# arkworks-rs/gemini

Hardware: AMD Instinct MI355X
Metric: BLS12-381 G1 MSM throughput (higher is better)
Workload: dtype u32x12 Montgomery Fq (381-bit integer), u32x8 Fr; 1 GPU; 2^20 G1 MSM per GPU (BASELINE configs[1]: 2^20 G1 MSM on one MI355X); pairs_per_gpu=1048576

## Files before the change

gemini_amd/csrc/msm.hip:

```cpp
#include <algorithm>
#include <atomic>
#include <chrono>
#include <condition_variable>
#include <cstdlib>
#include <cstring>
#include <functional>
#include <sched.h>
#include <cstdio>
#include <thread>
#include <vector>

#include "ctx.hpp"
#include "g1.cuh"
#include "host_field.hpp"

namespace gm {

constexpr uint32_t KEY_INV = 0xffffffffu;
constexpr int XYZZ_BYTES = 192;
constexpr int AFF_BYTES = 96;

struct DigitIter {
  uint32_t s[8];
  uint32_t carry;
// ... 316 lines not shown
  const uint32_t per = (G + 1023u) / 1024u;
  uint32_t v[4], nb[4], sa = 0, sb = 0;
  for (uint32_t k = 0; k < per; k++) {
    const uint32_t g = tid * per + k;
    v[k] = g < G ? gcount[g] : 0u;
    nb[k] = (v[k] + SORT_CH - 1u) / SORT_CH;
    sa += v[k];
    sb += nb[k];
  }
  a[tid] = sa;
  b[tid] = sb;
  __syncthreads();
  for (uint32_t d = 1; d < 1024; d <<= 1) {
    uint32_t xa = tid >= d ? a[tid - d] : 0, xb = tid >= d ? b[tid - d] : 0;
    __syncthreads();
    a[tid] += xa;
    b[tid] += xb;
    __syncthreads();
  }
  uint32_t ra = a[tid] - sa, rb = b[tid] - sb;
  for (uint32_t k = 0; k < per; k++) {
    const uint32_t g = tid * per + k;
    if (g < G) {
      goff[g] = ra;
      gcursor[g] = ra;
      blkoff[g] = rb;
    }
    ra += v[k];
    rb += nb[k];
  }
  if (tid == 1023) {
    goff[G] = a[1023];
    blkoff[G] = b[1023];
  }
}

template <bool SCATTER>
__global__ __launch_bounds__(256) void k_sort2(const uint64_t* __restrict__ tmp, const uint32_t* __restrict__ goff,
                                               const uint32_t* __restrict__ blkoff, SortGeom sg,
                                               uint32_t* __restrict__ counts_or_cursor, uint64_t* __restrict__ entries) {
  __shared__ uint32_t cnt[SORT_FMAX];
  __shared__ uint32_t base[SCATTER ? SORT_FMAX : 1];
  __shared__ uint32_t s_g;
  const uint32_t nf = 1u << sg.FB;
  if (blockIdx.x >= blkoff[sg.G]) return;
  if (threadIdx.x == 0) {
    uint32_t lo = 0, hi = sg.G;
    while (hi - lo > 1) {
      uint32_t mid = (lo + hi) >> 1;
      if (blkoff[mid] <= blockIdx.x) lo = mid; else hi = mid;
    }
    s_g = lo;
  }
  for (uint32_t f = threadIdx.x; f < nf; f += 256) cnt[f] = 0;
  __syncthreads();
  const uint32_t g = s_g;
  const uint32_t chunk = blockIdx.x - blkoff[g];
  const uint32_t lo = goff[g] + chunk * SORT_CH;
  const uint32_t hi = min(lo + SORT_CH, goff[g + 1]);
  const uint32_t mask = nf - 1u;
  for (uint32_t i0 = lo; i0 < hi; i0 += 256) {
    const uint32_t i = i0 + threadIdx.x;
    wave_atomic_inc(cnt, i < hi ? ((uint32_t)(tmp[i] >> 32) & mask) : KEY_INV);
  }
  __syncthreads();
  if (!SCATTER) {
    for (uint32_t f = threadIdx.x; f < nf; f += 256)
      if (cnt[f]) atomicAdd(counts_or_cursor + ((size_t)g << sg.FB) + f, cnt[f]);
    return;
  }
  for (uint32_t f = threadIdx.x; f < nf; f += 256) {
    const uint32_t k = cnt[f];
    if (SCATTER) base[f] = k ? atomicAdd(counts_or_cursor + ((size_t)g << sg.FB) + f, k) : 0u;
    cnt[f] = 0;
  }
  __syncthreads();
  for (uint32_t i0 = lo; i0 < hi; i0 += 256) {
    const uint32_t i = i0 + threadIdx.x;
    const bool live = i < hi;
    const uint64_t e = live ? tmp[i] : 0;
    const uint32_t f = (uint32_t)(e >> 32) & mask;
    const uint32_t r = wave_atomic_inc(cnt, live ? f : KEY_INV);
    if (live) entries[(SCATTER ? base[f] : 0u) + r] = e;
  }
}

constexpr uint32_t SORT_STAGE_FMAX = 2048;
__global__ __launch_bounds__(1024) void k_sort2_staged(const uint64_t* __restrict__ tmp, const uint32_t* __restrict__ goff,
                                                       const uint32_t* __restrict__ blkoff, SortGeom sg, uint32_t* __restrict__ cursor,
                                                       uint64_t* __restrict__ entries) {
  __shared__ uint64_t buf[SORT_CH];
  __shared__ uint32_t cnt[SORT_STAGE_FMAX], base[SORT_STAGE_FMAX], lst[SORT_STAGE_FMAX];
  __shared__ uint32_t scan[1024];
  __shared__ uint32_t s_g;
  const uint32_t tid = threadIdx.x;
  const uint32_t nf = 1u << sg.FB;
  if (blockIdx.x >= blkoff[sg.G]) return;
  if (tid == 0) {
    uint32_t lo = 0, hi = sg.G;
    while (hi - lo > 1) {
      uint32_t mid = (lo + hi) >> 1;
      if (blkoff[mid] <= blockIdx.x) lo = mid; else hi = mid;
    }
    s_g = lo;
  }
  for (uint32_t f = tid; f < nf; f += 1024) cnt[f] = 0;
  __syncthreads();
  const uint32_t g = s_g;
  const uint32_t chunk = blockIdx.x - blkoff[g];
  const uint32_t lo = goff[g] + chunk * SORT_CH;
  const uint32_t hi = min(lo + SORT_CH, goff[g + 1]);
  const uint32_t m = hi - lo;
  const uint32_t mask = nf - 1u;
  constexpr uint32_t PER = SORT_CH / 1024;
  uint64_t e[PER];
#pragma unroll
  for (uint32_t k = 0; k < PER; k++) {
    const uint32_t i = tid + k * 1024;
    e[k] = i < m ? tmp[lo + i] : 0;
    wave_atomic_inc(cnt, i < m ? ((uint32_t)(e[k] >> 32) & mask) : KEY_INV);
  }
  __syncthreads();
  const uint32_t per = nf > 1024 ? nf / 1024 : 1;
  uint32_t s = 0;
  for (uint32_t k = 0; k < per; k++) {
    const uint32_t f = tid * per + k;
    if (f < nf) {
      const uint32_t c = cnt[f];
      base[f] = c ? atomicAdd(cursor + ((size_t)g << sg.FB) + f, c) : 0u;
      s += c;
    }
  }
  scan[tid] = s;
  __syncthreads();
  for (uint32_t d = 1; d < 1024; d <<= 1) {
    const uint32_t x = tid >= d ? scan[tid - d] : 0;
    __syncthreads();
    scan[tid] += x;
    __syncthreads();
  }
  uint32_t run = scan[tid] - s;
  for (uint32_t k = 0; k < per; k++) {
    const uint32_t f = tid * per + k;
    if (f < nf) {
      lst[f] = run;
      run += cnt[f];
    }
  }
  __syncthreads();
  for (uint32_t f = tid; f < nf; f += 1024) cnt[f] = 0;
  __syncthreads();
#pragma unroll
  for (uint32_t k = 0; k < PER; k++) {
    const uint32_t i = tid + k * 1024;
    const uint32_t f = (uint32_t)(e[k] >> 32) & mask;
    const uint32_t r = wave_atomic_inc(cnt, i < m ? f : KEY_INV);
    if (i < m) buf[lst[f] + r] = e[k];
  }
  __syncthreads();
  for (uint32_t i = tid; i < m; i += 1024) {
    const uint64_t v = buf[i];
    const uint32_t f = (uint32_t)(v >> 32) & mask;
    entries[base[f] + (i - lst[f])] = v;
  }
}

// ... 340 lines not shown
          ebuf[2 * q][threadIdx.x] = ((uint64_t)v.y << 32) | v.x;
          ebuf[2 * q + 1][threadIdx.x] = ((uint64_t)v.w << 32) | v.z;
        }
      }
      return ebuf[k8][threadIdx.x];
    };
    auto base_of = [&](uint64_t e) {
      long long idx;
      if (tab_stride) {
        const uint32_t lo = (uint32_t)e & 0x7fffffffu;
        idx = (long long)(lo >> ENTRY_W_SHIFT) * tab_stride + first + step * (long long)(lo & ((1u << ENTRY_W_SHIFT) - 1u));
      } else {
        idx = first + step * (long long)(e & 0x3fffffffull);
      }
      const uint8_t* src = (phi != nullptr && ((e >> ENTRY_HALF_SHIFT) & 1ull)) ? phi : bases;
      return reinterpret_cast<const gm_u4v*>(src + (size_t)idx * AFF_BYTES);
    };
    uint64_t e = entry_at(start);
    const gm_u4v* bp = base_of(e);
    gm_u4v x0 = bp[0], x1 = bp[1], x2 = bp[2], y0 = bp[3], y1 = bp[4], y2 = bp[5];
    for (uint64_t i = start; i < end; i++) {
      uint64_t en = 0;
      gm_u4v n0 = x0, n1 = x1, n2 = x2, n3 = y0, n4 = y1, n5 = y2;
      if (i + 1 < end) {
        en = entry_at(i + 1);
        const gm_u4v* np = base_of(en);
        asm volatile(
            "global_load_dwordx4 %0, %6, off\n\t"
            "global_load_dwordx4 %1, %6, off offset:16\n\t"
            "global_load_dwordx4 %2, %6, off offset:32\n\t"
            "global_load_dwordx4 %3, %6, off offset:48\n\t"
            "global_load_dwordx4 %4, %6, off offset:64\n\t"
            "global_load_dwordx4 %5, %6, off offset:80"
            : "=&v"(n0), "=&v"(n1), "=&v"(n2), "=&v"(n3), "=&v"(n4), "=&v"(n5)
            : "v"(np));
      }
      const uint32_t key = (uint32_t)(e >> 32);
      if (key != cur) {
        if (cur != KEY_INV) {
          if (first_run) {
            head_key = cur;
            acc30_store(pp + (size_t)(2 * (size_t)t) * XYZZ30_BYTES, acc);
            first_run = false;
          } else {
            acc30_store(buckets + (size_t)cur * XYZZ30_BYTES, acc);
          }
        }
        cur = key;
        acc30_set_identity(acc);
      }
      const uint32_t nz = x0.x | x0.y | x0.z | x0.w | x1.x | x1.y | x1.z | x1.w | x2.x | x2.y | x2.z | x2.w | y0.x | y0.y | y0.z | y0.w |
                          y1.x | y1.y | y1.z | y1.w | y2.x | y2.y | y2.z | y2.w;
      if (nz != 0) {
        const uint32_t neg = (uint32_t)(e >> 31) & 1u;
        (void)g1_madd30_asm(acc, x0, x1, x2, y0, y1, y2, neg);
      }
      asm volatile("s_waitcnt vmcnt(0)" : "+v"(n0), "+v"(n1), "+v"(n2), "+v"(n3), "+v"(n4), "+v"(n5));
      e = en;
      x0 = n0; x1 = n1; x2 = n2; y0 = n3; y1 = n4; y2 = n5;
    }
    if (first_run) {
      head_key = cur;
      acc30_store(pp + (size_t)(2 * (size_t)t) * XYZZ30_BYTES, acc);
    } else {
      tail_key = cur;
      acc30_store(pp + (size_t)(2 * (size_t)t + 1) * XYZZ30_BYTES, acc);
    }
  }
  pk[2 * (size_t)t] = head_key;
  pk[2 * (size_t)t + 1] = tail_key;
  if (t == 0 && clk != nullptr) {
    clk[0] = (unsigned long long)(clock64() - clk_c0);
    clk[1] = (unsigned long long)(wall_clock64() - clk_w0);
  }
}

#ifdef GM_EXPERIMENTS
#include "msm_levels.inc"
#endif

__global__ __launch_bounds__(64) void k_merge(const uint32_t* __restrict__ keys_in, const uint8_t* __restrict__ pts_in,
                                              uint32_t E, uint32_t* __restrict__ keys_out,
                                              uint8_t* __restrict__ pts_out, uint8_t* __restrict__ buckets,
                                              int final_level) {
  __shared__ __attribute__((aligned(16))) uint8_t lds[128 * XYZZ30_BYTES];
  const int lane = threadIdx.x;
  const uint32_t wave = blockIdx.x;
  const uint32_t s0 = wave * 128u + 2u * lane;
  uint32_t hk = s0 < E ? keys_in[s0] : KEY_INV;
  uint32_t tk = s0 + 1 < E ? keys_in[s0 + 1] : KEY_INV;
  uint32_t hs = 2 * lane, ts = 2 * lane + 1;
  auto copy_rec = [](void* dst, const void* src) {
    const gm_u4v* s = reinterpret_cast<const gm_u4v*>(src);
    gm_u4v* d = reinterpret_cast<gm_u4v*>(dst);
#pragma unroll
    for (int i = 0; i < 13; i++) d[i] = s[i];
  };
  auto add_slots = [&](uint32_t dst_slot, uint32_t src_slot, Acc30& a) {
    Acc30 o;
    acc30_load(a, lds + dst_slot * XYZZ30_BYTES);
    acc30_load(o, lds + src_slot * XYZZ30_BYTES);
    acc30_add(a, o);
  };
  if (hk != KEY_INV) copy_rec(lds + hs * XYZZ30_BYTES, pts_in + (size_t)s0 * XYZZ30_BYTES);
  if (tk != KEY_INV) copy_rec(lds + ts * XYZZ30_BYTES, pts_in + ((size_t)s0 + 1) * XYZZ30_BYTES);
  if (hk == KEY_INV && tk != KEY_INV) {
    hk = tk;
    hs = ts;
    tk = KEY_INV;
  }
  __syncthreads();
  if (hk != KEY_INV && hk == tk) {
    Acc30 a;
    add_slots(hs, ts, a);
    acc30_store(lds + hs * XYZZ30_BYTES, a);
    tk = KEY_INV;
  }
  __syncthreads();

  {
    const uint32_t nhk = __shfl_down(hk, 1), nhs = __shfl_down(hs, 1), ntk = __shfl_down(tk, 1);
    const uint32_t ptk = __shfl_up(tk, 1);
    const bool give = lane < 63 && tk != KEY_INV && ntk != KEY_INV && nhk == tk;
    const bool taken = lane > 0 && tk != KEY_INV && ptk != KEY_INV && ptk == hk;
    if (__any(give)) {
      if (give) {
        Acc30 a;
        add_slots(ts, nhs, a);
        acc30_store(buckets + (size_t)tk * XYZZ30_BYTES, a);
      }
    }
    __syncthreads();
    if (taken) {
      hk = tk; hs = ts; tk = KEY_INV;
    }
    if (give) {
      if (taken) { hk = KEY_INV; } else { tk = KEY_INV; }
    }
  }

  for (int d = 1; d < 64; d <<= 1) {
    const uint32_t bhk = __shfl_down(hk, d), bhs = __shfl_down(hs, d);
    const uint32_t btk = __shfl_down(tk, d), bts = __shfl_down(ts, d);
    const bool act = (lane & (2 * d - 1)) == 0;
    bool do_add = false;
    uint32_t add_dst = 0, add_src = 0;
    uint32_t f1k = KEY_INV, f1s = 0, f2k = KEY_INV, f2s = 0;
    if (act && bhk != KEY_INV) {
      if (hk == KEY_INV) {
        hk = bhk; hs = bhs; tk = btk; ts = bts;
      } else {
        const bool a_two = tk != KEY_INV, b_two = btk != KEY_INV;
        const uint32_t alk = a_two ? tk : hk, als = a_two ? ts : hs;
        if (alk == bhk) {
          do_add = true; add_dst = als; add_src = bhs;
          if (b_two) {
            if (a_two) { f1k = alk; f1s = als; }
            tk = btk; ts = bts;
          }
        } else {
          if (a_two) { f1k = tk; f1s = ts; }
          if (b_two) { f2k = bhk; f2s = bhs; tk = btk; ts = bts; }
          else { tk = bhk; ts = bhs; }
        }
      }
    }
    if (__any(do_add)) {
      if (do_add) {
        Acc30 a;
        add_slots(add_dst, add_src, a);
        acc30_store(lds + add_dst * XYZZ30_BYTES, a);
      }
    }
    if (f1k != KEY_INV) copy_rec(buckets + (size_t)f1k * XYZZ30_BYTES, lds + f1s * XYZZ30_BYTES);
    if (f2k != KEY_INV) copy_rec(buckets + (size_t)f2k * XYZZ30_BYTES, lds + f2s * XYZZ30_BYTES);
    __syncthreads();
  }
  if (lane == 0) {
    if (final_level) {
      if (hk != KEY_INV) copy_rec(buckets + (size_t)hk * XYZZ30_BYTES, lds + hs * XYZZ30_BYTES);
      if (tk != KEY_INV) copy_rec(buckets + (size_t)tk * XYZZ30_BYTES, lds + ts * XYZZ30_BYTES);
    } else {
      keys_out[2 * (size_t)wave] = hk;
      keys_out[2 * (size_t)wave + 1] = tk;
      if (hk != KEY_INV) copy_rec(pts_out + (size_t)(2 * (size_t)wave) * XYZZ30_BYTES, lds + hs * XYZZ30_BYTES);
      if (tk != KEY_INV) copy_rec(pts_out + (size_t)(2 * (size_t)wave + 1) * XYZZ30_BYTES, lds + ts * XYZZ30_BYTES);
    }
  }
}

enum { GS_STRIDED = 0, GS_PLANE = 1 };
struct GroupSumArgs {
  const uint8_t* in;
  uint8_t* out;
  int mode;
  uint32_t n_out;
  uint32_t per_win;
  uint32_t win_stride;
  uint32_t n_lo, s_hi, s_lo, s_e, len;
  uint32_t nb;
  uint32_t lpo_shift;
  int out_canonical;
  const uint32_t* in_cnt;
};
struct GroupSumJobs {
  GroupSumArgs j[3];
  uint32_t blk_end[3];
  const uint32_t* err_src;
  uint32_t* err_dst;
  const unsigned long long* clk_src;
};

__global__ __launch_bounds__(256) void k_group_sum(GroupSumJobs J) {
  if (J.err_dst && blockIdx.x == 0 && threadIdx.x == 0) {
    *J.err_dst = *J.err_src;
    if (J.clk_src) {
      unsigned long long* d = reinterpret_cast<unsigned long long*>(J.err_dst + 2);
      d[0] = J.clk_src[0];
      d[1] = J.clk_src[1];
    }
  }
  const int job = blockIdx.x < J.blk_end[0] ? 0 : (blockIdx.x < J.blk_end[1] ? 1 : 2);
  const GroupSumArgs& a = J.j[job];
  const uint32_t blk0 = job == 0 ? 0u : J.blk_end[job - 1];
  const uint8_t* __restrict__ in = a.in;
  uint8_t* __restrict__ out = a.out;
  const uint32_t gt = (blockIdx.x - blk0) * blockDim.x + threadIdx.x;
  const uint32_t lpo = 1u << a.lpo_shift;
  const uint32_t o = gt >> a.lpo_shift, q = gt & (lpo - 1u);
  Acc30 acc;
  acc30_zero(acc);
  const uint32_t* __restrict__ in_cnt = a.in_cnt;
  auto filled = [&](size_t slot) { return in_cnt == nullptr || in_cnt[slot] != 0u; };
  auto add_rec = [&](size_t slot) {
    if (!filled(slot)) return;
    Acc30 v;
    acc30_load(v, in + slot * XYZZ30_BYTES);
    acc30_add(acc, v);
  };
  auto load_first = [&](size_t slot) {
    if (filled(slot)) acc30_load(acc, in + slot * XYZZ30_BYTES);
  };
  if (o < a.n_out) {
    const uint32_t w = o / a.per_win, r = o % a.per_win;
    const size_t base = (size_t)w * a.win_stride;
    if (a.mode == GS_STRIDED) {
      const size_t b0 = base + (size_t)(r / a.n_lo) * a.s_hi + (size_t)(r % a.n_lo) * a.s_lo;
      if (q < a.len) load_first(b0 + (size_t)q * a.s_e);
      for (uint32_t e = q + lpo; e < a.len; e += lpo) add_rec(b0 + (size_t)e * a.s_e);
    } else {
      const uint32_t nb = a.nb;
      if (r == nb) {
        const uint32_t cnt0 = nb ? (1u << (nb - 1)) : 1u;
        if (q < cnt0) load_first(base + 2u * q);
        for (uint32_t e = q + lpo; e < cnt0; e += lpo) add_rec(base + 2u * e);
      } else {
        const uint32_t half = nb ? (1u << (nb - 1)) : 0u;
        auto slot_of = [&](uint32_t e) { return ((e >> r) << (r + 1)) | (1u << r) | (e & ((1u << r) - 1u)); };
        if (q < half) load_first(base + slot_of(q));
        for (uint32_t e = q + lpo; e < half; e += lpo) add_rec(base + slot_of(e));
      }
    }
  }
#pragma unroll 1
  for (int m = (int)(lpo >> 1); m >= 1; m >>= 1) {
    Acc30 other;
    acc30_shfl_xor(other, acc, m);
    acc30_add(acc, other);
  }
  if (o < a.n_out && q == 0) {
// ... 639 lines not shown
  size_t tab_n = 0;
  static const bool fuse_tables_env = !(getenv("GM_MSM_FUSE_TABLES") && atoi(getenv("GM_MSM_FUSE_TABLES")) == 0);
  if (multi && multi->block && !C->msm_c_override && fuse_tables_env) {
    auto covers = [&](size_t tn) {
      for (int l = 0; l < multi->levels; l++) {
        const int64_t lo = multi->start[l], hi = multi->start[l] + step * (int64_t)(multi->n[l] - 1);
        if (lo < 0 || hi < 0 || (size_t)lo >= tn || (size_t)hi >= tn) return false;
      }
      return tn <= ((size_t)1 << ENTRY_W_SHIFT);
    };
    if (bases->table != nullptr && bases->tab_c <= 20 && covers(bases->n)) {
      tab_ptr = bases->table;
      tab_c_sel = bases->tab_c;
      tab_n = bases->n;
    } else {
      for (const Bases::TableSet& ts : bases->extra)
        if (ts.c <= 20 && ts.c >= 18 && covers(ts.n)) {
          tab_ptr = ts.t;
          tab_c_sel = ts.c;
          tab_n = ts.n;
          break;
        }
    }
  }
  if (!multi && !C->msm_c_override && n < ((size_t)1 << ENTRY_W_SHIFT)) {
    if (bases->table != nullptr && n >= tab_min) {
      tab_ptr = bases->table;
      tab_c_sel = bases->tab_c;
      tab_n = bases->n;
    } else if (C->msm_table_min <= ((size_t)1 << 17) || n >= C->msm_table_min) {
      const int64_t last = first + step * (int64_t)(n - 1);
      for (const Bases::TableSet& ts : bases->extra)
        if (n >= ts.min_n && n < ts.max_n && first >= 0 && last >= 0 && (size_t)first < ts.n && (size_t)last < ts.n) {
          tab_ptr = ts.t;
          tab_c_sel = ts.c;
          tab_n = ts.n;
          break;
        }
    }
  }
  const bool use_table = tab_ptr != nullptr;
  const bool multi_block = multi && multi->block;
  static const int fuse_c_env = getenv("GM_MSM_FUSE_C") ? atoi(getenv("GM_MSM_FUSE_C")) : 16;
  const int c = multi ? (multi_block ? (use_table ? tab_c_sel : fuse_c_env) : 8) : (use_table ? tab_c_sel : (C->msm_c_override ? C->msm_c_override : choose_window(n)));
  GM_CHECK(c >= 2 && c <= 22, GM_EINVAL, "msm: window width %d out of range [2, 22]", c);
  static const bool sort_atomic_env0 = getenv("GM_MSM_SORT") && !strcmp(getenv("GM_MSM_SORT"), "atomic");
  static const int acc0_waves = getenv("GM_ACC0_WAVES") ? atoi(getenv("GM_ACC0_WAVES")) : 2;
  const size_t bucket_bytes = XYZZ30_BYTES;
  const bool use_glv = GM_GLV(1) && !multi && bases->phi != nullptr && !use_table && C->msm_affine_levels == 0 && !sort_atomic_env0 && n <= ((size_t)1 << 26);
  const int W = ((use_glv ? 128 : 256) + c - 1) / c;
  GM_CHECK(nparts == 1 || !use_table, GM_EINVAL, "msm: the fixed-base table path is not split into window groups");
  const int w_lo = part * W / nparts, Wg = (part + 1) * W / nparts - w_lo;
  const uint32_t B = 1u << (c - 1);
  const int Wb = multi ? multi->levels * (use_table ? 1 : W) : (use_table ? 1 : Wg);
  const size_t nbuckets = (size_t)Wb * B;
  const uint8_t* d_bases = use_table ? tab_ptr : bases->d;
  const long long tab_stride = use_table ? (long long)tab_n : 0;
  const uint64_t Nall = (uint64_t)n * (uint64_t)W * (use_glv ? 2u : 1u);
  const uint64_t N = (uint64_t)n * (uint64_t)(use_table ? W : Wg) * (use_glv ? 2u : 1u);
  GM_CHECK(Nall < (1ull << 32), GM_EINVAL, "msm: n*W = %llu entries exceed 2^32; chunk the stream", (unsigned long long)Nall);

  int levels = C->msm_affine_levels;
  if (levels < 0) {
    levels = 0;
    if (N >= ((uint64_t)1 << 22))
      for (uint64_t avg = N / nbuckets; avg >= 8 && levels < 6; avg >>= 1) levels++;
  }
  GM_CHECK(levels <= 8, GM_EINVAL, "msm: %d affine levels (max 8)", levels);
  uint64_t Nacc = N;
  for (int l = 0; l < levels; l++) Nacc = Nacc / 2 + 2 * nbuckets + 2;

  static const int L_env = getenv("GM_MSM_L") ? atoi(getenv("GM_MSM_L")) : 0;
  const uint64_t Nacc_all = nparts > 1 ? Nall : Nacc;
  const uint64_t lanes0 = Nacc_all >= ((uint64_t)1 << 24) ? 262144 : 131072;
  static const uint64_t L_cap = getenv("GM_MSM_LCAP") ? (uint64_t)atoi(getenv("GM_MSM_LCAP")) : 256;
  uint32_t L = (uint32_t)std::min<uint64_t>(L_cap, std::max<uint64_t>(4, (Nacc_all + lanes0 - 1) / lanes0));
  if (L_env > 0) L = (uint32_t)L_env;
  L = (L + 1u) & ~1u;
  const uint64_t T0 = (Nacc + L - 1) / L;
  const uint64_t T0pad = (T0 + 255) / 256 * 256;
  const uint64_t E1 = 2 * T0pad;

  int rc;
  const size_t counts_words = (nbuckets + 2 + SORT_GMAX + 1 + 63) / 64 * 64;
  if ((rc = ws.counts.ensure(counts_words * 4))) return rc;
  if ((rc = ws.offsets.ensure((nbuckets + 1) * 4))) return rc;
  if ((rc = ws.cursor.ensure((nbuckets + 1) * 4))) return rc;
  if ((rc = ws.misc.ensure((nbuckets / SCAN_PER_BLOCK + 2) * 4))) return rc;
  if ((rc = ws.entries.ensure(N * 8))) return rc;
  if ((rc = ws.buckets.ensure(nbuckets * bucket_bytes))) return rc;
  if ((rc = ws.pk[0].ensure(E1 * 4))) return rc;
  if ((rc = ws.pp[0].ensure(E1 * bucket_bytes))) return rc;
  const uint64_t E2 = 2 * ((E1 + 127) / 128);
  if ((rc = ws.pk[1].ensure(E2 * 4))) return rc;
  if ((rc = ws.pp[1].ensure(E2 * bucket_bytes))) return rc;

  const uint32_t* sc = reinterpret_cast<const uint32_t*>(d_scalars);
  GM_HIP(hipMemsetAsync(ws.counts.p, 0, counts_words * 4, st));
  uint32_t* d_err = ws.counts.as<uint32_t>() + nbuckets + 1;
  const bool bucket_counts_valid = levels == 0;
  if (!bucket_counts_valid) GM_HIP(hipMemsetAsync(ws.buckets.p, 0, nbuckets * bucket_bytes, st));
  const uint32_t dblocks = (uint32_t)((n + 255) / 256);
  Profiler& pf = C->prof;
  auto run_scan = [&]() {
    const uint32_t nb = (uint32_t)((nbuckets + SCAN_PER_BLOCK - 1) / SCAN_PER_BLOCK);
    hipLaunchKernelGGL(k_scan_block_sums, dim3(nb), dim3(256), 0, st, ws.counts.as<uint32_t>(), (uint32_t)nbuckets,
                       ws.misc.as<uint32_t>());
    hipLaunchKernelGGL(k_scan_top, dim3(1), dim3(1024), 0, st, ws.misc.as<uint32_t>(), nb,
                       ws.offsets.as<uint32_t>() + nbuckets);
    hipLaunchKernelGGL(k_scan_apply, dim3(nb), dim3(256), 0, st, ws.counts.as<uint32_t>(), (uint32_t)nbuckets,
                       ws.misc.as<uint32_t>(), ws.offsets.as<uint32_t>(), ws.cursor.as<uint32_t>());
  };
  static const bool sort_atomic_env = getenv("GM_MSM_SORT") && !strcmp(getenv("GM_MSM_SORT"), "atomic");
  static const bool sort_flat_env = !(getenv("GM_MSM_SORT") && !strcmp(getenv("GM_MSM_SORT"), "blocks"));
  const bool sort_atomic = sort_atomic_env && !use_table && nparts == 1 && !multi_block;
  const bool sort_flat = sort_flat_env && !sort_atomic && !use_table && nparts == 1 && !multi_block && N <= ((uint64_t)1 << 21) && nbuckets <= ((size_t)1 << 18);
  LevelGeom lg{};
  if (multi_block) {
    lg.levels = multi->levels;
    lg.step = (int)step;
    uint32_t at = 0;
    for (int l = 0; l < multi->levels; l++) {
      lg.start[l] = at;
      lg.scal[l] = reinterpret_cast<const uint32_t*>(multi->scalars[l]);
      lg.base0[l] = (long long)multi->start[l];
      at += (uint32_t)multi->n[l];
    }
    lg.start[multi->levels] = at;
  }
  if (multi && !multi_block) {
    MultiGeom mg{};
    mg.c = c;
    mg.W = W;
    mg.levels = multi->levels;
    mg.step = (int)step;
    mg.B = B;
    for (int j = 0; j + 1 < W; j++) {
      const int b = c * j + c - 1;
      if (b < 256) mg.K[b >> 5] |= 1u << (b & 31);
    }
    uint32_t at = 0;
    for (int l = 0; l < multi->levels; l++) {
      mg.start[l] = at;
      mg.scal[l] = reinterpret_cast<const uint32_t*>(multi->scalars[l]);
      mg.base0[l] = (long long)multi->start[l];
      at += (uint32_t)multi->n[l];
    }
    mg.start[multi->levels] = at;
    GM_CHECK(N <= ((uint64_t)1 << 21) && nbuckets <= ((size_t)1 << 18), GM_EINVAL, "msm: fused calls too large for the flat sort (%llu entries, %zu buckets)",
             (unsigned long long)N, nbuckets);
    const dim3 grid((uint32_t)((n + 255) / 256), (uint32_t)W);
    pf.begin(part, PROF_DIGITS, st);
    hipLaunchKernelGGL(k_digits_multi<false>, grid, dim3(256), 0, st, mg, mont, ws.counts.as<uint32_t>(), (uint64_t*)nullptr, d_err);
    hipLaunchKernelGGL(k_scan_small, dim3(1), dim3(1024), 0, st, ws.counts.as<uint32_t>(), (uint32_t)nbuckets, ws.offsets.as<uint32_t>(),
                       ws.cursor.as<uint32_t>());
    pf.end(part, PROF_DIGITS, st);
    pf.begin(part, PROF_SCATTER, st);
    hipLaunchKernelGGL(k_digits_multi<true>, grid, dim3(256), 0, st, mg, mont, ws.cursor.as<uint32_t>(), ws.entries.as<uint64_t>(), d_err);
    pf.end(part, PROF_SCATTER, st);
  } else if (sort_flat) {
    FlatGeom fg{};
    fg.c = c;
    fg.W = W;
    fg.glv = use_glv ? 1 : 0;
    fg.B = B;
    for (int j = 0; j + 1 < W; j++) {
      const int b = c * j + c - 1;
      if (b < 256) fg.K[b >> 5] |= 1u << (b & 31);
    }
    const dim3 grid((uint32_t)((n + 255) / 256), (uint32_t)(W * (use_glv ? 2 : 1)));
    pf.begin(part, PROF_DIGITS, st);
    hipLaunchKernelGGL(k_digits_flat<false>, grid, dim3(256), 0, st, sc, (uint32_t)n, mont, fg, ws.counts.as<uint32_t>(), (uint64_t*)nullptr, d_err);
    hipLaunchKernelGGL(k_scan_small, dim3(1), dim3(1024), 0, st, ws.counts.as<uint32_t>(), (uint32_t)nbuckets, ws.offsets.as<uint32_t>(),
                       ws.cursor.as<uint32_t>());
    pf.end(part, PROF_DIGITS, st);
    pf.begin(part, PROF_SCATTER, st);
    hipLaunchKernelGGL(k_digits_flat<true>, grid, dim3(256), 0, st, sc, (uint32_t)n, mont, fg, ws.cursor.as<uint32_t>(), ws.entries.as<uint64_t>(), d_err);
    pf.end(part, PROF_SCATTER, st);
  } else if (sort_atomic) {
    pf.begin(part, PROF_DIGITS, st);
    hipLaunchKernelGGL(k_msm_digits<false>, dim3(dblocks), dim3(256), 0, st, sc, (uint32_t)n, mont, c, W, B,
                       ws.counts.as<uint32_t>(), (uint64_t*)nullptr, d_err);
    pf.end(part, PROF_DIGITS, st);
    pf.begin(part, PROF_SCAN, st);
    run_scan();
    pf.end(part, PROF_SCAN, st);
    pf.begin(part, PROF_SCATTER, st);
    hipLaunchKernelGGL(k_msm_digits<true>, dim3(dblocks), dim3(256), 0, st, sc, (uint32_t)n, mont, c, W, B,
                       ws.cursor.as<uint32_t>(), ws.entries.as<uint64_t>(), d_err);
    pf.end(part, PROF_SCATTER, st);
  } else {
    SortGeom sg;
    sg.c = c;
    sg.W = W;
    sg.w_lo = use_table ? 0 : w_lo;
    sg.Wg = use_table ? W : Wg;
    sg.glv = use_glv ? 1 : 0;
    sg.B = B;
    sg.shared = use_table ? 1 : 0;
    sg.FB = std::min<uint32_t>((uint32_t)(c - 1), 10u);
    if (multi_block) sg.FB = std::min<uint32_t>((uint32_t)(c - 1), std::max<uint32_t>(sg.FB, 11u));
    while ((nbuckets >> sg.FB) > SORT_GMAX && (1u << sg.FB) < SORT_FMAX) sg.FB++;
    sg.G = (uint32_t)(nbuckets >> sg.FB);
    GM_CHECK(sg.G <= SORT_GMAX, GM_EINVAL, "msm: %u coarse sort bins exceed %u (window %d too wide for this sort)", sg.G, SORT_GMAX, c);
    if ((rc = ws.tmp_entries.ensure(N * 8))) return rc;
    if ((rc = ws.sortmeta.ensure((size_t)(3 * (sg.G + 1)) * 4))) return rc;
    uint32_t* gcount = ws.counts.as<uint32_t>() + nbuckets + 2;
    uint32_t* goff = ws.sortmeta.as<uint32_t>();
    uint32_t* gcursor = goff + (sg.G + 1);
    uint32_t* blkoff = gcursor + (sg.G + 1);
    const uint32_t b1 = (uint32_t)((n + SORT_TS - 1) / SORT_TS);
    const uint32_t b2 = (uint32_t)(N / SORT_CH + sg.G + 1);
    pf.begin(part, PROF_DIGITS, st);
    hipLaunchKernelGGL(k_sort1<false>, dim3(b1), dim3(256), 0, st, sc, (uint32_t)n, mont, sg, lg, gcount, (uint64_t*)nullptr, d_err);
    hipLaunchKernelGGL(k_sort1_scan, dim3(1), dim3(1024), 0, st, gcount, sg.G, goff, gcursor, blkoff);
    const size_t stage1_lds = (size_t)SORT_TS * sg.Wg * (use_glv ? 2 : 1) * 8 + (size_t)3 * sg.G * 4 + 1024 * 4;
    static const bool sort1_staged_env = !(getenv("GM_MSM_SORT1") && !strcmp(getenv("GM_MSM_SORT1"), "direct"));
    if (sort1_staged_env && sg.Wg * (use_glv ? 2 : 1) <= SORT1_STAGE_WMAX && stage1_lds <= 160 * 1024) {
      static bool attr_set = false;
      if (!attr_set) {
        GM_HIP(hipFuncSetAttribute(reinterpret_cast<const void*>(k_sort1_staged), hipFuncAttributeMaxDynamicSharedMemorySize, 160 * 1024));
        attr_set = true;
      }
      hipLaunchKernelGGL(k_sort1_staged, dim3(b1), dim3(1024), stage1_lds, st, sc, (uint32_t)n, mont, sg, lg, gcursor, ws.tmp_entries.as<uint64_t>());
    } else {
      hipLaunchKernelGGL(k_sort1<true>, dim3(b1), dim3(256), 0, st, sc, (uint32_t)n, mont, sg, lg, gcursor, ws.tmp_entries.as<uint64_t>(), d_err);
    }
    pf.end(part, PROF_DIGITS, st);
    pf.begin(part, PROF_SCATTER, st);
    hipLaunchKernelGGL(k_sort2<false>, dim3(b2), dim3(256), 0, st, ws.tmp_entries.as<uint64_t>(), goff, blkoff, sg,
                       ws.counts.as<uint32_t>(), (uint64_t*)nullptr);
    run_scan();
    static const bool sort_staged = !(getenv("GM_MSM_SORT2") && !strcmp(getenv("GM_MSM_SORT2"), "direct"));
    if (sort_staged && (1u << sg.FB) <= SORT_STAGE_FMAX)
      hipLaunchKernelGGL(k_sort2_staged, dim3(b2), dim3(1024), 0, st, ws.tmp_entries.as<uint64_t>(), goff, blkoff, sg,
                         ws.cursor.as<uint32_t>(), ws.entries.as<uint64_t>());
    else
      hipLaunchKernelGGL(k_sort2<true>, dim3(b2), dim3(256), 0, st, ws.tmp_entries.as<uint64_t>(), goff, blkoff, sg,
                         ws.cursor.as<uint32_t>(), ws.entries.as<uint64_t>());
    pf.end(part, PROF_SCATTER, st);
  }
  const uint64_t* acc_entries = ws.entries.as<uint64_t>();
  const uint32_t* acc_total = ws.offsets.as<uint32_t>() + nbuckets;
  const uint8_t* acc_bases = d_bases;
  long long acc_first = (long long)first, acc_step = multi ? 1ll : (long long)step, acc_tab = tab_stride;
#ifdef GM_EXPERIMENTS
#define GM_MSM_LEVELS_HOST 1
#include "msm_levels.inc"
#undef GM_MSM_LEVELS_HOST
#else
  GM_CHECK(levels == 0, GM_EINVAL, "msm: affine tree levels are an experiment of round 2; rebuild with -DGM_EXPERIMENTS (DESIGN.md section 8)");
#endif
  if (!ws.have_done_ev) {
    for (int e = 0; e < MSM_SLOTS; e++) GM_HIP(hipEventCreateWithFlags(&ws.done_ev[e], hipEventDisableTiming));
    GM_HIP(hipEventCreateWithFlags(&ws.sort_ev, hipEventDisableTiming));
    GM_HIP(hipEventCreateWithFlags(&ws.acc_ev, hipEventDisableTiming));
    ws.have_done_ev = true;
  }
  if (sts.acc != st) {
    GM_HIP(hipEventRecord(ws.sort_ev, st));
    GM_HIP(hipStreamWaitEvent(sts.acc, ws.sort_ev, 0));
  }
  st = sts.acc;
  pf.begin(part, PROF_ACC0, st);
  static const size_t acc0_lds_pad = getenv("GM_ACC0_LDS_PAD") ? (size_t)strtoull(getenv("GM_ACC0_LDS_PAD"), nullptr, 10) : 0;
  if ((rc = ws.clk.ensure(16))) return rc;
  unsigned long long* acc_clk = ws.clk.as<unsigned long long>();
  static const int acc0_pf_env = getenv("GM_ACC0_PREFETCH") ? atoi(getenv("GM_ACC0_PREFETCH")) : -1;
  const bool acc0_pf = acc0_pf_env >= 0 ? acc0_pf_env != 0 : use_table;
  if (acc0_pf)
    hipLaunchKernelGGL(k_acc0_pf<2>, dim3((uint32_t)(T0pad / 256)), dim3(256), 0, st, acc_entries, acc_total, acc_bases, acc_first, acc_step,
                       acc_tab, L, ws.pk[0].as<uint32_t>(), ws.pp[0].as<uint8_t>(), ws.buckets.as<uint8_t>(), use_glv ? bases->phi : (const uint8_t*)nullptr, acc_clk);
  else if (acc0_waves == 2)
    hipLaunchKernelGGL(k_acc0<2>, dim3((uint32_t)(T0pad / 256)), dim3(256), acc0_lds_pad, st, acc_entries, acc_total, acc_bases, acc_first, acc_step,
                       acc_tab, L, ws.pk[0].as<uint32_t>(), ws.pp[0].as<uint8_t>(), ws.buckets.as<uint8_t>(), use_glv ? bases->phi : (const uint8_t*)nullptr, acc_clk);
  else
    hipLaunchKernelGGL(k_acc0<3>, dim3((uint32_t)(T0pad / 256)), dim3(256), 0, st, acc_entries, acc_total, acc_bases, acc_first, acc_step,
                       acc_tab, L, ws.pk[0].as<uint32_t>(), ws.pp[0].as<uint8_t>(), ws.buckets.as<uint8_t>(), use_glv ? bases->phi : (const uint8_t*)nullptr, acc_clk);
  pf.end(part, PROF_ACC0, st);
  if (sts.tail != st) {
    GM_HIP(hipEventRecord(ws.acc_ev, st));
    GM_HIP(hipStreamWaitEvent(sts.tail, ws.acc_ev, 0));
  }
  st = sts.tail;
  pf.begin(part, PROF_MERGE, st);
  {
    uint64_t E = E1;
    int src = 0;
    for (;;) {
      uint32_t waves = (uint32_t)((E + 127) / 128);
      int final_level = waves == 1;
      hipLaunchKernelGGL(k_merge, dim3(waves), dim3(64), 0, st, ws.pk[src].as<uint32_t>(), ws.pp[src].as<uint8_t>(),
                         (uint32_t)E, ws.pk[src ^ 1].as<uint32_t>(), ws.pp[src ^ 1].as<uint8_t>(),
                         ws.buckets.as<uint8_t>(), final_level);
      if (final_level) break;
      E = 2ull * waves;
      src ^= 1;
    }
  }

  pf.end(part, PROF_MERGE, st);
  pf.begin(part, PROF_REDUCE, st);
  const uint32_t nbits = (uint32_t)(c - 1);
  uint32_t wf[3] = {0, 0, 0};
  int m;
  static const int fields_env = getenv("GM_MSM_FIELDS") ? atoi(getenv("GM_MSM_FIELDS")) : 0;
  if (nbits <= 7) {
    m = 1;
    wf[0] = nbits;
  } else if (nbits <= 14 || (fields_env == 2 && nbits <= 16)) {
    m = 2;
    wf[0] = nbits / 2;
    wf[1] = nbits - wf[0];
  } else {
    m = 3;
    static const bool odd_low = !(getenv("GM_MSM_ODD_BIT") && !strcmp(getenv("GM_MSM_ODD_BIT"), "high"));
    wf[0] = odd_low ? (nbits + 2) / 3 : nbits / 3;
    wf[1] = (nbits - wf[0]) / 2;
    wf[2] = nbits - wf[0] - wf[1];
  }
  static const int lpo_env = getenv("GM_MSM_LPO_LOG") ? atoi(getenv("GM_MSM_LPO_LOG")) : 0;
  const int lpo_target_log = lpo_env ? lpo_env : (nbuckets >= ((size_t)1 << 21) ? 18 : 17);
  uint32_t lpo_jobs = 1;
  auto lpo_for = [&](uint32_t len, uint32_t n_out) {
    uint32_t s = 0;
    while (s < 5 && (1u << s) < len && ((uint64_t)n_out << s) * lpo_jobs < (1ull << lpo_target_log)) s++;
    return s;
  };
  const uint8_t* bucket_in = ws.buckets.as<uint8_t>();
  const uint32_t* bucket_cnt = bucket_counts_valid ? ws.counts.as<uint32_t>() : nullptr;
  auto strided = [&](const uint8_t* in, uint8_t* out, uint32_t win_in, uint32_t n_hi, uint32_t n_lo, uint32_t s_hi, uint32_t s_lo,
                     uint32_t s_e, uint32_t len) {
    GroupSumArgs g{};
    g.in = in; g.out = out; g.mode = GS_STRIDED; g.in_cnt = in == bucket_in ? bucket_cnt : nullptr;
    g.per_win = n_hi * n_lo; g.n_out = (uint32_t)Wb * g.per_win; g.win_stride = win_in;
    g.n_lo = n_lo; g.s_hi = s_hi; g.s_lo = s_lo; g.s_e = s_e; g.len = len; g.lpo_shift = lpo_for(len, g.n_out);
    return g;
  };
  auto plane = [&](const uint8_t* in, uint8_t* out, uint32_t nb) {
    GroupSumArgs g{};
    g.in = in; g.out = out; g.mode = GS_PLANE; g.out_canonical = 1;
    g.in_cnt = in == bucket_in ? bucket_cnt : nullptr;
    g.per_win = nb + 1; g.n_out = (uint32_t)Wb * g.per_win; g.win_stride = 1u << nb; g.nb = nb;
    g.lpo_shift = lpo_for(nb ? (1u << (nb - 1)) : 1u, g.n_out);
    return g;
  };
  uint8_t* planes = nullptr;
  size_t plane_count = 0;
  auto launch = [&](std::initializer_list<GroupSumArgs> jobs, bool last = false) {
    GroupSumJobs J{};
    if (last) {
      J.err_src = d_err;
      J.err_dst = reinterpret_cast<uint32_t*>(planes + plane_count * XYZZ_BYTES);
      J.clk_src = ws.clk.as<unsigned long long>();
    }
    uint32_t tot = 0;
    int k = 0;
    for (const GroupSumArgs& g : jobs) {
      J.j[k] = g;
      tot += (uint32_t)((((uint64_t)g.n_out << g.lpo_shift) + 255) / 256);
      J.blk_end[k] = tot;
      k++;
    }
    for (; k < 3; k++) J.blk_end[k] = tot;
    hipLaunchKernelGGL(k_group_sum, dim3(tot), dim3(256), 0, st, J);
  };
  size_t plane_off[3];
  for (int k = 0; k < m; k++) {
    plane_off[k] = plane_count;
    plane_count += (size_t)Wb * (wf[k] + 1);
  }
  const size_t plane_bytes = plane_count * XYZZ_BYTES + 24;
  if (ws.host_planes_cap[slot] < plane_bytes) {
    if (ws.host_planes[slot]) (void)hipHostFree(ws.host_planes[slot]);
    ws.host_planes[slot] = nullptr;
    ws.host_planes_cap[slot] = 0;
    GM_HIP(hipHostMalloc((void**)&ws.host_planes[slot], plane_bytes, hipHostMallocDefault));
// ... 743 lines not shown
```

Baseline: 349.3 Mscalar/s.

## Fuse sort2 bucket counting with per-group scan using last-block tickets

Replaces the separate sort2 count kernel and global scan launches with a single kernel. Each block counts its chunk's fine keys in LDS, adds them to global counts, and the last block per group (found through an atomic ticket) scans that group's counts into offsets and cursor. Spare blocks fill offsets for empty groups. This removes kernel launches and a global scan pass, at the cost of atomic tickets, a serialized tail scan per group and extra counter workspace.

```diff
diff --git a/gemini_amd/csrc/msm.hip b/gemini_amd/csrc/msm.hip
--- a/gemini_amd/csrc/msm.hip
+++ b/gemini_amd/csrc/msm.hip
@@ -422,6 +422,92 @@
     const uint32_t f = (uint32_t)(e >> 32) & mask;
     const uint32_t r = wave_atomic_inc(cnt, live ? f : KEY_INV);
     if (live) entries[(SCATTER ? base[f] : 0u) + r] = e;
+  }
+}
+
+__global__ __launch_bounds__(1024) void k_sort2_count_scan(const uint64_t* __restrict__ tmp, const uint32_t* __restrict__ goff,
+                                                           const uint32_t* __restrict__ blkoff, SortGeom sg, uint32_t* __restrict__ counts,
+                                                           uint32_t* __restrict__ tickets, uint32_t* __restrict__ offsets,
+                                                           uint32_t* __restrict__ cursor) {
+  __shared__ uint32_t cnt[SORT_FMAX];
+  __shared__ uint32_t scan[1024];
+  __shared__ uint32_t s_g, s_last;
+  const uint32_t tid = threadIdx.x;
+  const uint32_t nf = 1u << sg.FB;
+  const uint32_t nblk = blkoff[sg.G];
+  if (blockIdx.x >= nblk) {
+    const uint32_t nspare = gridDim.x - nblk, j = blockIdx.x - nblk;
+    for (uint32_t g = j; g < sg.G; g += nspare) {
+      const uint32_t o = goff[g];
+      if (goff[g + 1] != o) continue;
+      for (uint32_t f = tid; f < nf; f += 1024) {
+        offsets[((size_t)g << sg.FB) + f] = o;
+        cursor[((size_t)g << sg.FB) + f] = o;
+      }
+    }
+    if (j == 0 && tid == 0) offsets[(size_t)sg.G << sg.FB] = goff[sg.G];
+    return;
+  }
+  if (tid == 0) {
+    uint32_t lo = 0, hi = sg.G;
+    while (hi - lo > 1) {
+      uint32_t mid = (lo + hi) >> 1;
+      if (blkoff[mid] <= blockIdx.x) lo = mid; else hi = mid;
+    }
+    s_g = lo;
+  }
+  for (uint32_t f = tid; f < nf; f += 1024) cnt[f] = 0;
+  __syncthreads();
+  const uint32_t g = s_g;
+  const uint32_t chunk = blockIdx.x - blkoff[g];
+  const uint32_t lo = goff[g] + chunk * SORT_CH;
+  const uint32_t m = min(lo + SORT_CH, goff[g + 1]) - lo;
+  const uint32_t mask = nf - 1u;
+  const uint32_t* keys = reinterpret_cast<const uint32_t*>(tmp + lo) + 1;
+  constexpr uint32_t PER = SORT_CH / 1024;
+  uint32_t k[PER];
+#pragma unroll
+  for (uint32_t q = 0; q < PER; q++) {
+    const uint32_t i = tid + q * 1024;
+    k[q] = i < m ? keys[2 * (size_t)i] : 0u;
+  }
+#pragma unroll
+  for (uint32_t q = 0; q < PER; q++) wave_atomic_inc(cnt, tid + q * 1024 < m ? (k[q] & mask) : KEY_INV);
+  __syncthreads();
+  uint32_t* gc = counts + ((size_t)g << sg.FB);
+  for (uint32_t f = tid; f < nf; f += 1024)
+    if (cnt[f]) atomicAdd(gc + f, cnt[f]);
+  asm volatile("s_waitcnt vmcnt(0)" ::: "memory");
+  __syncthreads();
+  if (tid == 0) {
+    const uint32_t nchunks = blkoff[g + 1] - blkoff[g];
+    s_last = atomicAdd(tickets + g, 1u) == nchunks - 1u;
+  }
+  __syncthreads();
+  if (!s_last) return;
+  const uint32_t per = nf > 1024 ? nf / 1024 : 1;
+  uint32_t v[4], s = 0;
+  for (uint32_t q = 0; q < per; q++) {
+    const uint32_t f = tid * per + q;
+    v[q] = f < nf ? __hip_atomic_load(gc + f, __ATOMIC_RELAXED, __HIP_MEMORY_SCOPE_AGENT) : 0u;
+    s += v[q];
+  }
+  scan[tid] = s;
+  __syncthreads();
+  for (uint32_t d = 1; d < 1024; d <<= 1) {
+    const uint32_t x = tid >= d ? scan[tid - d] : 0;
+    __syncthreads();
+    scan[tid] += x;
+    __syncthreads();
+  }
+  uint32_t run = goff[g] + scan[tid] - s;
+  for (uint32_t q = 0; q < per; q++) {
+    const uint32_t f = tid * per + q;
+    if (f < nf) {
+      offsets[((size_t)g << sg.FB) + f] = run;
+      cursor[((size_t)g << sg.FB) + f] = run;
+      run += v[q];
+    }
   }
 }
 
@@ -1837,7 +1923,7 @@
   const uint64_t E1 = 2 * T0pad;
 
   int rc;
-  const size_t counts_words = (nbuckets + 2 + SORT_GMAX + 1 + 63) / 64 * 64;
+  const size_t counts_words = (nbuckets + 2 + 2 * SORT_GMAX + 1 + 63) / 64 * 64;
   if ((rc = ws.counts.ensure(counts_words * 4))) return rc;
   if ((rc = ws.offsets.ensure((nbuckets + 1) * 4))) return rc;
   if ((rc = ws.cursor.ensure((nbuckets + 1) * 4))) return rc;
@@ -1983,9 +2069,15 @@
     }
     pf.end(part, PROF_DIGITS, st);
     pf.begin(part, PROF_SCATTER, st);
-    hipLaunchKernelGGL(k_sort2<false>, dim3(b2), dim3(256), 0, st, ws.tmp_entries.as<uint64_t>(), goff, blkoff, sg,
-                       ws.counts.as<uint32_t>(), (uint64_t*)nullptr);
-    run_scan();
+    static const bool sort2_split_env = getenv("GM_MSM_SORT2_COUNT") && !strcmp(getenv("GM_MSM_SORT2_COUNT"), "split");
+    if (!sort2_split_env) {
+      hipLaunchKernelGGL(k_sort2_count_scan, dim3(b2), dim3(1024), 0, st, ws.tmp_entries.as<uint64_t>(), goff, blkoff, sg,
+                         ws.counts.as<uint32_t>(), gcount + SORT_GMAX, ws.offsets.as<uint32_t>(), ws.cursor.as<uint32_t>());
+    } else {
+      hipLaunchKernelGGL(k_sort2<false>, dim3(b2), dim3(256), 0, st, ws.tmp_entries.as<uint64_t>(), goff, blkoff, sg,
+                         ws.counts.as<uint32_t>(), (uint64_t*)nullptr);
+      run_scan();
+    }
     static const bool sort_staged = !(getenv("GM_MSM_SORT2") && !strcmp(getenv("GM_MSM_SORT2"), "direct"));
     if (sort_staged && (1u << sg.FB) <= SORT_STAGE_FMAX)
       hipLaunchKernelGGL(k_sort2_staged, dim3(b2), dim3(1024), 0, st, ws.tmp_entries.as<uint64_t>(), goff, blkoff, sg,
```

After: 349.5 Mscalar/s (median of 6 runs). Within noise of the previous version (+0.1%).

## Resolve merge tail with a pair-walk kernel and skip tree merge unless needed

Applied to the files above, without the earlier changes.

Adds a k_merge_pairs kernel in which each thread owning a bucket segment walks forward through consecutive accumulator pairs with the same key, sums up to eight parts, and writes the bucket directly. If any run is longer, it sets a device flag, and the existing multi-level k_merge tree runs only in that case (each launch returns early when the flag is zero). This aims to replace several serial merge launches with one flat pass in the common short-run case. The merge launches are still issued and must check the flag, and long runs fall back to the full tree after wasted work.

```diff
diff --git a/gemini_amd/csrc/msm.hip b/gemini_amd/csrc/msm.hip
--- a/gemini_amd/csrc/msm.hip
+++ b/gemini_amd/csrc/msm.hip
@@ -928,7 +928,8 @@
 __global__ __launch_bounds__(64) void k_merge(const uint32_t* __restrict__ keys_in, const uint8_t* __restrict__ pts_in,
                                               uint32_t E, uint32_t* __restrict__ keys_out,
                                               uint8_t* __restrict__ pts_out, uint8_t* __restrict__ buckets,
-                                              int final_level) {
+                                              int final_level, const uint32_t* __restrict__ run_flag) {
+  if (run_flag != nullptr && *run_flag == 0u) return;
   __shared__ __attribute__((aligned(16))) uint8_t lds[128 * XYZZ30_BYTES];
   const int lane = threadIdx.x;
   const uint32_t wave = blockIdx.x;
@@ -1032,6 +1033,46 @@
       if (hk != KEY_INV) copy_rec(pts_out + (size_t)(2 * (size_t)wave) * XYZZ30_BYTES, lds + hs * XYZZ30_BYTES);
       if (tk != KEY_INV) copy_rec(pts_out + (size_t)(2 * (size_t)wave + 1) * XYZZ30_BYTES, lds + ts * XYZZ30_BYTES);
     }
+  }
+}
+
+constexpr int MERGE_WALK_MAX = 8;
+__global__ __launch_bounds__(256) void k_merge_pairs(const uint32_t* __restrict__ pk, const uint8_t* __restrict__ pp, uint32_t T,
+                                                     uint8_t* __restrict__ buckets, uint32_t* __restrict__ run_flag) {
+  const uint32_t t = blockIdx.x * blockDim.x + threadIdx.x;
+  if (t >= T) return;
+  const uint32_t hk = pk[2 * (size_t)t], tk = pk[2 * (size_t)t + 1];
+  if (hk == KEY_INV) return;
+  bool head_owner = true;
+  if (t > 0) {
+    const uint32_t ptk = pk[2 * (size_t)t - 1];
+    head_owner = (ptk != KEY_INV ? ptk : pk[2 * (size_t)t - 2]) != hk;
+  }
+#pragma unroll 1
+  for (int seg = 0; seg < 2; seg++) {
+    const bool from_tail = seg == 1;
+    if (from_tail ? tk == KEY_INV : !head_owner) continue;
+    const uint32_t k = from_tail ? tk : hk;
+    uint32_t p = t;
+    Acc30 acc;
+    acc30_load(acc, pp + (2 * (size_t)p + (from_tail ? 1 : 0)) * XYZZ30_BYTES);
+    bool open = from_tail || tk == KEY_INV;
+    bool done = true;
+    int parts = 1;
+    while (open && p + 1 < T && pk[2 * (size_t)(p + 1)] == k) {
+      if (parts == MERGE_WALK_MAX) {
+        atomicOr(run_flag, 1u);
+        done = false;
+        break;
+      }
+      p++;
+      Acc30 o;
+      acc30_load(o, pp + (2 * (size_t)p) * XYZZ30_BYTES);
+      acc30_add(acc, o);
+      parts++;
+      open = pk[2 * (size_t)p + 1] == KEY_INV;
+    }
+    if (done) acc30_store(buckets + (size_t)k * XYZZ30_BYTES, acc);
   }
 }
 
@@ -1837,7 +1878,8 @@
   const uint64_t E1 = 2 * T0pad;
 
   int rc;
-  const size_t counts_words = (nbuckets + 2 + SORT_GMAX + 1 + 63) / 64 * 64;
+  const size_t merge_flag_word = nbuckets + 2 + SORT_GMAX + 1;
+  const size_t counts_words = (merge_flag_word + 1 + 63) / 64 * 64;
   if ((rc = ws.counts.ensure(counts_words * 4))) return rc;
   if ((rc = ws.offsets.ensure((nbuckets + 1) * 4))) return rc;
   if ((rc = ws.cursor.ensure((nbuckets + 1) * 4))) return rc;
@@ -2039,15 +2081,21 @@
   }
   st = sts.tail;
   pf.begin(part, PROF_MERGE, st);
+  static const bool tail_old = getenv("GM_MSM_TAIL") && !strcmp(getenv("GM_MSM_TAIL"), "old");
+  uint32_t* merge_flag = ws.counts.as<uint32_t>() + merge_flag_word;
   {
     uint64_t E = E1;
     int src = 0;
+    const bool pairs = !tail_old && E1 > 128;
+    if (pairs)
+      hipLaunchKernelGGL(k_merge_pairs, dim3((uint32_t)((E1 / 2 + 255) / 256)), dim3(256), 0, st, ws.pk[0].as<uint32_t>(), ws.pp[0].as<uint8_t>(),
+                         (uint32_t)(E1 / 2), ws.buckets.as<uint8_t>(), merge_flag);
     for (;;) {
       uint32_t waves = (uint32_t)((E + 127) / 128);
       int final_level = waves == 1;
       hipLaunchKernelGGL(k_merge, dim3(waves), dim3(64), 0, st, ws.pk[src].as<uint32_t>(), ws.pp[src].as<uint8_t>(),
                          (uint32_t)E, ws.pk[src ^ 1].as<uint32_t>(), ws.pp[src ^ 1].as<uint8_t>(),
-                         ws.buckets.as<uint8_t>(), final_level);
+                         ws.buckets.as<uint8_t>(), final_level, pairs ? (const uint32_t*)merge_flag : nullptr);
       if (final_level) break;
       E = 2ull * waves;
       src ^= 1;
```

Result: no change. 345.2 Mscalar/s before, 349.3 Mscalar/s after, median of 6 (+1.2%).
